# kepengxu/PGTFormer

Measured on NVIDIA H100. Metric: clips_per_s, higher is better.
Workload: dtype bf16

## Files before the change

pgtformer_b200/csrc/gemm_tc.cu:

```cuda
#include <cudaTypedefs.h>
#include <cstdio>
#include <cstdlib>

#include "common.cuh"
#include "tmap.cuh"
#include "ptx.cuh"
#include "epi_common.cuh"

namespace pgt {

constexpr int BM = 128;
constexpr int BK = 64;
constexpr int EPI_WARPS = 8;
constexpr int GEMM_THREADS = EPI_WARPS * 32 + 128;
constexpr int PRODUCER_WARP = EPI_WARPS;
constexpr int DMA_WARP = EPI_WARPS + 1;
constexpr int CONSUMER_REGS = 232;
constexpr int PRODUCER_REGS = 40;
static_assert(2 * 128 * CONSUMER_REGS + 128 * PRODUCER_REGS <= 65536, "register file");
constexpr int XCH_LD = 68;
constexpr int XCH_BYTES = BM * XCH_LD * 4;
constexpr int XCH_WG_LD = 36;
constexpr int XCH_WG_BYTES = BM * XCH_WG_LD * 4;
constexpr int EPI_BAR = 1;
constexpr int PP_XCH_BAR = 2;
constexpr int PP_MMA_BAR = 4;
constexpr int PP_EPI_BAR = 6;
constexpr int A_STAGE_BYTES = BM * BK * 2;
constexpr int PANEL_BYTES = BM * 128;
template <int BN>
constexpr int staging_slots() { return BN == 256 ? 2 : 4; }
constexpr int PREFETCH_TILES = 2;

enum { MODE_LINEAR = 0, MODE_CONV_S1 = 1, MODE_CONV_S2 = 2 };

struct GemmParams {
  int mode;
  int M, N, K;
  int num_kb, m_tiles, n_tiles;
  int F, H, W;
  int tw, th, tn, tiles_x, tiles_y;
  int cin_blocks, ksize, pad_lo, cin_ld;
  int pad_x, pad_y;
  long long o_sx, o_sy, o_sf;
  int b_resident;
  int fast_epi;
  int has_res_map;
  const float* bias;
  int act, epi_mode;
  float* gn_stats;
  int gn_cpg;
  int ntaps, tap_kw, tap_oy, tap_ox;
  int gn_tpf;
  int gn_fstride;
  int relu_after_res;
  const void* residual;
  int ldr, res_dtype;
  const void* aux;
  int ldaux;
  float sft_w;
  void* out;
  int ldo, out_dtype, out_layout;
  double flops;
};

template <int BN>
struct GemmCfg {
  static constexpr int B_STAGE_BYTES = BN * BK * 2;
  static constexpr int STAGE_BYTES = A_STAGE_BYTES + B_STAGE_BYTES;
  static constexpr int SLOTS = staging_slots<BN>();
  static constexpr int STAGING_BYTES = SLOTS * PANEL_BYTES;
  static constexpr int BUDGET = 232448 - 1024  - STAGING_BYTES - XCH_BYTES - 256 ;
  static constexpr int STAGES = (BUDGET / STAGE_BYTES) > 6 ? 6 : (BUDGET / STAGE_BYTES);
  static constexpr int SMEM_BYTES = STAGES * STAGE_BYTES + STAGING_BYTES + XCH_BYTES + 256 + 1024;
  static_assert(SMEM_BYTES <= 232448, "gemm smem budget");
};

__device__ __forceinline__ void tile_mn(const GemmParams& p, int tile, int& m_blk, int& n_blk) {
  n_blk = tile % p.n_tiles;
  m_blk = tile / p.n_tiles;
}


__device__ __forceinline__ void decode_conv_tile(const GemmParams& p, int m_blk, int& n0, int& y0, int& x0) {
  const int tx = m_blk % p.tiles_x;
  const int t2 = m_blk / p.tiles_x;
  const int ty = t2 % p.tiles_y;
  const int tf = t2 / p.tiles_y;
  x0 = tx * p.tw;
  y0 = ty * p.th;
  n0 = tf * p.tn;
}

template <int N>
__device__ __forceinline__ void act_chunk(float (&f)[N], int act) {
  switch (act) {
    case PGT_ACT_GELU:
#pragma unroll
      for (int j = 0; j < N; ++j) f[j] = gelu_erf(f[j]);
      break;
    case PGT_ACT_SILU:
#pragma unroll
      for (int j = 0; j < N; ++j) f[j] = apply_act(f[j], PGT_ACT_SILU);
      break;
    case PGT_ACT_LRELU02:
#pragma unroll
      for (int j = 0; j < N; ++j) f[j] = fmaxf(f[j], 0.2f * f[j]);
      break;
    case PGT_ACT_RELU:
#pragma unroll
      for (int j = 0; j < N; ++j) f[j] = fmaxf(f[j], 0.f);
      break;
    case PGT_ACT_SIGMOID:
#pragma unroll
      for (int j = 0; j < N; ++j) f[j] = apply_act(f[j], PGT_ACT_SIGMOID);
      break;
    default: break;
  }
}

struct EpiCtx {
  uint8_t* staging;
  float* xch;
  uint64_t* res_bar;
  uint64_t* slot_ready;
};

__device__ __forceinline__ uint4 lds128(uint32_t a) {
  uint4 u;
  asm volatile("ld.shared.v4.b32 {%0, %1, %2, %3}, [%4];" : "=r"(u.x), "=r"(u.y), "=r"(u.z), "=r"(u.w) : "r"(a) : "memory");
  return u;
}
__device__ __forceinline__ void sts128(uint32_t a, const uint4& u) {
  asm volatile("st.shared.v4.b32 [%0], {%1, %2, %3, %4};" ::"r"(a), "r"(u.x), "r"(u.y), "r"(u.z), "r"(u.w) : "memory");
}

template <bool kSft>
__device__ __forceinline__ void epi_finish(const GemmParams& p, const uint32_t (&v)[32], const float* bias32, uint32_t srow,
                                           int r, int sub, int esize, bool has_res, float* gq, int gcol,
                                           const float4 (&pre)[8], bool use_pre) {
  float f[32];
  if (use_pre) {
#pragma unroll
    for (int q = 0; q < 8; ++q) {
      f[4 * q + 0] = __uint_as_float(v[4 * q + 0]) + pre[q].x;
      f[4 * q + 1] = __uint_as_float(v[4 * q + 1]) + pre[q].y;
      f[4 * q + 2] = __uint_as_float(v[4 * q + 2]) + pre[q].z;
      f[4 * q + 3] = __uint_as_float(v[4 * q + 3]) + pre[q].w;
    }
  } else if (bias32 != nullptr) {
    const float4* b4 = reinterpret_cast<const float4*>(bias32);
#pragma unroll
    for (int q = 0; q < 8; ++q) {
      const float4 bb = __ldg(b4 + q);
      f[4 * q + 0] = __uint_as_float(v[4 * q + 0]) + bb.x;
      f[4 * q + 1] = __uint_as_float(v[4 * q + 1]) + bb.y;
      f[4 * q + 2] = __uint_as_float(v[4 * q + 2]) + bb.z;
      f[4 * q + 3] = __uint_as_float(v[4 * q + 3]) + bb.w;
    }
  } else {
#pragma unroll
    for (int i = 0; i < 32; ++i) f[i] = __uint_as_float(v[i]);
    if (p.bias != nullptr) {
#pragma unroll
      for (int i = 0; i < 32; ++i)
        if (gcol + i < p.N) f[i] += __ldg(p.bias + gcol + i);
    }
  }
  if (p.act != PGT_ACT_NONE && !p.relu_after_res) act_chunk(f, p.act);
  if (esize == 2) {
    uint32_t off[4];
#pragma unroll
    for (int q = 0; q < 4; ++q) off[q] = srow + ((((sub << 2) + q) ^ (r & 7)) << 4);
    if (has_res) {
      uint4 ur[4];
#pragma unroll
      for (int q = 0; q < 4; ++q) ur[q] = lds128(off[q]);
      if (kSft) {
        uint4 ux[4];
#pragma unroll
        for (int q = 0; q < 4; ++q) ux[q] = lds128(off[q] + PANEL_BYTES);
#pragma unroll
        for (int q = 0; q < 4; ++q) {
          const float2 a = unpack_bf16x2(ur[q].x), b = unpack_bf16x2(ur[q].y), c = unpack_bf16x2(ur[q].z), d = unpack_bf16x2(ur[q].w);
          const float rr[8] = {a.x, a.y, b.x, b.y, c.x, c.y, d.x, d.y};
          const float2 sa = unpack_bf16x2(ux[q].x), sb = unpack_bf16x2(ux[q].y), sc = unpack_bf16x2(ux[q].z), sd = unpack_bf16x2(ux[q].w);
          const float ss[8] = {sa.x, sa.y, sb.x, sb.y, sc.x, sc.y, sd.x, sd.y};
// ... 34 lines not shown
    }
  } else {
    if (has_res) {
      uint4 ur[8];
#pragma unroll
      for (int q = 0; q < 8; ++q) ur[q] = lds128(srow + ((q ^ (r & 7)) << 4));
#pragma unroll
      for (int q = 0; q < 8; ++q) {
        f[4 * q + 0] += __uint_as_float(ur[q].x); f[4 * q + 1] += __uint_as_float(ur[q].y);
        f[4 * q + 2] += __uint_as_float(ur[q].z); f[4 * q + 3] += __uint_as_float(ur[q].w);
      }
    }
    if (p.relu_after_res) {
#pragma unroll
      for (int e = 0; e < 32; ++e) f[e] = fmaxf(f[e], 0.f);
    }
#pragma unroll
    for (int q = 0; q < 8; ++q) {
      uint4 o;
      o.x = __float_as_uint(f[4 * q]); o.y = __float_as_uint(f[4 * q + 1]);
      o.z = __float_as_uint(f[4 * q + 2]); o.w = __float_as_uint(f[4 * q + 3]);
      sts128(srow + ((q ^ (r & 7)) << 4), o);
    }
  }
}

struct ItemCursor {
  int tile, pnl;
};

template <int BN>
struct ItemStream {
  const GemmParams& p;
  int num_tiles, PW, panels_total;
  __device__ ItemStream(const GemmParams& pp, int nt) : p(pp), num_tiles(nt) {
    PW = 128 / (pp.out_dtype == PGT_BF16 ? 2 : 4);
    panels_total = BN / PW;
  }
  __device__ int panels_in_tile(int t) const {
    int mb, nb;
    tile_mn(p, t, mb, nb);
    const int cb = nb * BN;
    const int n = (p.N - cb + PW - 1) / PW;
    return n > panels_total ? panels_total : n;
  }
  __device__ bool valid(const ItemCursor& c) const { return c.tile < num_tiles; }
  __device__ void next(ItemCursor& c) const {
    if (++c.pnl >= panels_in_tile(c.tile)) { c.tile += gridDim.x; c.pnl = 0; }
  }
};

template <int BN>
__device__ __forceinline__ void epilogue_dma_loop(const GemmParams& p, const EpiCtx& ctx, const CUtensorMap& tmO,
                                                  const CUtensorMap& tmR, const CUtensorMap& tmX, int lane, int num_tiles) {
  if (!p.fast_epi) return;
  const ItemStream<BN> is(p, num_tiles);
  constexpr int SLOTS = staging_slots<BN>();
  static_assert(SLOTS == 4 || SLOTS == 2, "ring positions are computed with shifts");
  const bool sft = SLOTS == 4 && p.epi_mode == PGT_EPI_SFT;
  const int S = sft ? 2 : 1;
  const int R = SLOTS / S;
  auto coords = [&](const ItemCursor& c, int& col, int& m_blk, int& n0, int& y0, int& x0) {
    int nb;
    tile_mn(p, c.tile, m_blk, nb);
    col = nb * BN + c.pnl * is.PW;
    n0 = y0 = x0 = 0;
    if (p.mode != MODE_LINEAR) decode_conv_tile(p, m_blk, n0, y0, x0);
  };
  auto prepare = [&](const ItemCursor& c, int pos) {
    uint64_t* bar = &ctx.res_bar[pos];
    if (!p.has_res_map) { mbar_arrive(bar); return; }
    int col, m_blk, n0, y0, x0;
    coords(c, col, m_blk, n0, y0, x0);
    uint8_t* dst = ctx.staging + pos * S * PANEL_BYTES;
    mbar_arrive_expect_tx(bar, S * PANEL_BYTES);
    if (p.mode == MODE_LINEAR) {
      tma_load_2d(dst, &tmR, bar, col, m_blk * BM);
      if (sft) tma_load_2d(dst + PANEL_BYTES, &tmX, bar, col, m_blk * BM);
    } else {
      tma_load_4d(dst, &tmR, bar, col, x0, y0, n0);
      if (sft) tma_load_4d(dst + PANEL_BYTES, &tmX, bar, col, x0, y0, n0);
    }
  };
  ItemCursor cp{(int)blockIdx.x, 0}, cs{(int)blockIdx.x, 0};
  if (lane == 0) {
    for (int i = 0; i < R && is.valid(cp); ++i) { prepare(cp, i); is.next(cp); }
  }
  __syncwarp();
  const int rshift = R == 4 ? 2 : 1;
  for (int k = 0; is.valid(cs); ++k, is.next(cs)) {
    const int pos = k & (R - 1);
    mbar_wait(&ctx.slot_ready[pos], (k >> rshift) & 1);
    if (lane == 0) {
      int col, m_blk, n0, y0, x0;
      coords(cs, col, m_blk, n0, y0, x0);
      const uint8_t* src = ctx.staging + pos * S * PANEL_BYTES;
      if (p.mode == MODE_LINEAR) tma_store_2d(&tmO, src, col, m_blk * BM);
      else tma_store_4d(&tmO, src, col, x0, y0, n0);
      bulk_commit();
      if (k >= 1 && is.valid(cp)) {
        bulk_wait_read<1>();
        prepare(cp, (k - 1) & (R - 1));
        is.next(cp);
      }
    }
    __syncwarp();
  }
  if (lane == 0) bulk_wait0();
}

struct DirectRow {
// ... 130 lines not shown
          mbar_wait_spin(&ctx.res_bar[pos], (k >> 1) & 1);
          const int col0 = col_base + pnl * PW + half * 32;
          uint32_t v[32];
          smem_row_32(xrow + half * 32, v);
          float4 nb[8];
          epi_finish<true>(p, v, bias_vec ? p.bias + col0 : nullptr, stg + pos * 2 * PANEL_BYTES, r, half, esize, true,
                           gn_ptr(col0), col0, nb, false);
          fence_proxy_async();
          mbar_arrive(&ctx.slot_ready[pos]);
          ++k;
        }
      } else {
        for (int pp = 0; pp < 64 / PW; ++pp) {
          const int pnl = g * (64 / PW) + pp;
          if (pnl >= npan) break;
          const int pos = k & (SLOTS - 1);
          const bool mine = (nsub == 2) || ((pnl & 1) == half);
          const int sb = (nsub == 2) ? half : 0;
          const int col0 = col_base + pnl * PW + sb * 32;
          float4 b[8];
          const bool pre = BN < 256 && bias_vec;
          if (mine && pre) {
            const float4* gb = reinterpret_cast<const float4*>(p.bias + col0);
#pragma unroll
            for (int q = 0; q < 8; ++q) b[q] = __ldg(gb + q);
          }
          mbar_wait_spin(&ctx.res_bar[pos], (k >> SLOT_SHIFT) & 1);
          if (mine) {
            uint32_t v[32];
            smem_row_32(xrow + pnl * PW + sb * 32 - g * 64, v);
            epi_finish<false>(p, v, bias_vec && !pre ? p.bias + col0 : nullptr, stg + pos * PANEL_BYTES, r, sb, esize,
                              p.has_res_map != 0, gn_ptr(col0), col0, b, pre);
          }
          fence_proxy_async();
          mbar_arrive(&ctx.slot_ready[pos]);
          ++k;
        }
      }
    } else {
      const int c0 = g * 64 + half * 32;
      if (drow.valid) {
#pragma unroll 1
        for (int sc16 = 0; sc16 < 32; sc16 += 16) {
          const int col0 = col_base + c0 + sc16;
          if (col0 >= p.N) break;
          epi_direct16<kVec>(p, drow, xrow + half * 32 + sc16, col0);
        }
      }
      __syncwarp();
    }
  });
}

template <int BN, bool kVec>
__device__ __forceinline__ void epilogue_tile_wg(const GemmParams& p, const EpiCtx& ctx, int wq, int bar, int tile, int k,
                                                 const float (&acc)[2][BN / 2]) {
  const int lane = lane_id();
  const int r = wq * 32 + lane;
  const int esize = (p.out_dtype == PGT_BF16) ? 2 : 4;
  const ItemStream<BN> is(p, 0);
  const int nsub = is.PW / 32;
  constexpr int SLOTS = staging_slots<BN>();
  constexpr int SLOT_SHIFT = SLOTS == 4 ? 2 : 1;
  const bool sft = SLOTS == 4 && p.epi_mode == PGT_EPI_SFT;
  const bool bias_vec = kVec && p.bias != nullptr && (p.N % 32) == 0;
  const float* xrow = ctx.xch + r * XCH_WG_LD;

  int n_blk, m_blk;
  tile_mn(p, tile, m_blk, n_blk);
  const int col_base = n_blk * BN;
  const int npan = p.fast_epi ? is.panels_in_tile(tile) : 0;
  const uint32_t stg = smem_u32(ctx.staging) + r * 128;
  const DirectRow drow = p.fast_epi ? DirectRow{false, 0, 0, 0, 0} : direct_row(p, m_blk, r);

  static_for<0, BN / 32>([&](auto cc) {
    constexpr int c = decltype(cc)::value;
    const int pnl = c / nsub, sub = c - pnl * nsub;
    if (p.fast_epi && pnl >= npan) return;
    const int col0 = col_base + c * 32;
    if (col0 < p.N) {
      named_bar_sync(bar, 128);
      acc_to_smem<c * 32, 32>(acc[0], ctx.xch, XCH_WG_LD, wq, lane);
      acc_to_smem<c * 32, 32>(acc[1], ctx.xch + 64 * XCH_WG_LD, XCH_WG_LD, wq, lane);
      named_bar_sync(bar, 128);
    }
    if (p.fast_epi) {
      const int item = k + pnl;
      const int pos = sft ? (item & 1) : (item & (SLOTS - 1));
      if (sub == 0) mbar_wait_spin(&ctx.res_bar[pos], sft ? ((item >> 1) & 1) : ((item >> SLOT_SHIFT) & 1));
      if (col0 < p.N) {
        uint32_t v[32];
        smem_row_32(xrow, v);
        float4 nb[8];
        if (sft)
          epi_finish<true>(p, v, bias_vec ? p.bias + col0 : nullptr, stg + pos * 2 * PANEL_BYTES, r, sub, esize, true,
                           gn_stats_ptr(p, m_blk, wq, col0), col0, nb, false);
        else
          epi_finish<false>(p, v, bias_vec ? p.bias + col0 : nullptr, stg + pos * PANEL_BYTES, r, sub, esize,
                            p.has_res_map != 0, gn_stats_ptr(p, m_blk, wq, col0), col0, nb, false);
      }
      if (sub == nsub - 1) {
        fence_proxy_async();
        mbar_arrive(&ctx.slot_ready[pos]);
      }
    } else if (col0 < p.N) {
      if (drow.valid) {
#pragma unroll 1
        for (int sc16 = 0; sc16 < 32; sc16 += 16) {
          if (col0 + sc16 >= p.N) break;
          epi_direct16<kVec>(p, drow, xrow + sc16, col0 + sc16);
        }
      }
      __syncwarp();
    }
  });
}

__device__ __forceinline__ void release_stage(uint64_t* bar, int lane) {
  __syncwarp();
  if (lane == 0) mbar_arrive(bar);
}

template <int BN, bool kVec>
__global__ void __launch_bounds__(GEMM_THREADS, 1)
gemm_tc_kernel(const __grid_constant__ CUtensorMap tmA, const __grid_constant__ CUtensorMap tmB,
               const __grid_constant__ CUtensorMap tmO, const __grid_constant__ CUtensorMap tmR,
               const __grid_constant__ CUtensorMap tmX, const GemmParams p) {
  using Cfg = GemmCfg<BN>;
  constexpr int STAGES = Cfg::STAGES;
  extern __shared__ uint8_t smem_raw[];
  uint8_t* smem = reinterpret_cast<uint8_t*>((reinterpret_cast<uintptr_t>(smem_raw) + 1023) & ~uintptr_t(1023));
  uint8_t* smem_a = smem;
  uint8_t* smem_b = smem + STAGES * A_STAGE_BYTES;
  uint8_t* staging = smem + STAGES * Cfg::STAGE_BYTES;
  float* xch = reinterpret_cast<float*>(staging + Cfg::STAGING_BYTES);
  uint64_t* bars = reinterpret_cast<uint64_t*>(staging + Cfg::STAGING_BYTES + XCH_BYTES);
  uint64_t* full_bar = bars;
  uint64_t* empty_bar = bars + STAGES;
  uint64_t* res_bar = bars + 2 * STAGES;
  uint64_t* slot_ready = res_bar + Cfg::SLOTS;

  const int warp = threadIdx.x >> 5;
  const int lane = threadIdx.x & 31;
  const int num_tiles = p.m_tiles * p.n_tiles;

  if (warp == PRODUCER_WARP && lane == 0) {
    tma_prefetch_desc(&tmA);
    tma_prefetch_desc(&tmB);
    if (p.fast_epi) tma_prefetch_desc(&tmO);
    if (p.has_res_map) tma_prefetch_desc(&tmR);
    if (p.fast_epi && p.epi_mode == PGT_EPI_SFT) tma_prefetch_desc(&tmX);
    for (int i = 0; i < STAGES; ++i) {
      mbar_init(&full_bar[i], 1);
      mbar_init(&empty_bar[i], EPI_WARPS);
    }
    for (int i = 0; i < Cfg::SLOTS; ++i) {
      mbar_init(&res_bar[i], 1);
      mbar_init(&slot_ready[i], EPI_WARPS * 32);
    }
    fence_barrier_init();
  }
  __syncthreads();

  if (warp >= EPI_WARPS) {
    setmaxnreg_dec<PRODUCER_REGS>();
    if (warp == PRODUCER_WARP) {
      int stage = 0;
      uint32_t phase = 0;
      for (int tile = blockIdx.x; tile < num_tiles; tile += gridDim.x) {
        int n_blk, m_blk;
        tile_mn(p, tile, m_blk, n_blk);
        int n0 = 0, y0 = 0, x0 = 0;
        if (p.mode != MODE_LINEAR) decode_conv_tile(p, m_blk, n0, y0, x0);
        for (int kb = 0; kb < p.num_kb; ++kb) {
          mbar_wait(&empty_bar[stage], phase ^ 1);
          if (elect_one()) {
            void* dst_a = smem_a + stage * A_STAGE_BYTES;
            void* dst_b = smem_b + stage * Cfg::B_STAGE_BYTES;
            int cb = 0, ax = 0, ay = 0, a5 = 0;
            if (p.mode != MODE_LINEAR) {
              const int tap = kb / p.cin_blocks;
              cb = kb - tap * p.cin_blocks;
              const int dy = tap / p.ksize;
              const int dx = tap - dy * p.ksize;
              if (p.mode == MODE_CONV_S1) {
                ax = x0 + dx - p.pad_x; ay = y0 + dy - p.pad_y;
              } else {
                const int oy = dy - p.pad_lo, ox = dx - p.pad_lo;
                const int qy = (oy < 0) ? -((1 - oy) >> 1) : (oy >> 1);
                const int qx = (ox < 0) ? -((1 - ox) >> 1) : (ox >> 1);
                const int py = oy - 2 * qy, px = ox - 2 * qx;
                cb = px * p.cin_ld + cb * BK;
                ax = x0 + qx; ay = y0 + qy; a5 = py;
              }
            }
            mbar_arrive_expect_tx(&full_bar[stage], Cfg::STAGE_BYTES);
            if (p.mode == MODE_LINEAR) tma_load_2d(dst_a, &tmA, &full_bar[stage], kb * BK, m_blk * BM);
            else if (p.mode == MODE_CONV_S1) tma_load_4d(dst_a, &tmA, &full_bar[stage], cb * BK, ax, ay, n0);
            else tma_load_5d(dst_a, &tmA, &full_bar[stage], cb, ax, a5, ay, n0);
            tma_load_2d(dst_b, &tmB, &full_bar[stage], kb * BK, n_blk * BN);
          }
          __syncwarp();
          if (++stage == STAGES) { stage = 0; phase ^= 1; }
        }
      }
      for (int i = 0; i < STAGES; ++i) {
        mbar_wait(&empty_bar[stage], phase ^ 1);
        if (++stage == STAGES) { stage = 0; phase ^= 1; }
      }
    } else if (warp == DMA_WARP) {
      const EpiCtx ctx{staging, xch, res_bar, slot_ready};
      epilogue_dma_loop<BN>(p, ctx, tmO, tmR, tmX, lane, num_tiles);
    }
  } else {
    setmaxnreg_inc<CONSUMER_REGS>();
    const EpiCtx ctx{staging, xch, res_bar, slot_ready};
    const int wg = warp >> 2;
    const uint32_t a_rows = smem_u32(smem_a) + wg * 64 * 128;
    const uint32_t b_base = smem_u32(smem_b);
    int stage = 0;
    uint32_t phase = 0;
    int k = 0;
    for (int tile = blockIdx.x; tile < num_tiles; tile += gridDim.x) {
      float acc[BN / 2];
      int prev = -1;
      for (int kb = 0; kb < p.num_kb; ++kb) {
        mbar_wait_spin(&full_bar[stage], phase);
        const uint64_t da = wgmma_desc_k_sw128(a_rows + stage * A_STAGE_BYTES);
        const uint64_t db = wgmma_desc_k_sw128(b_base + stage * Cfg::B_STAGE_BYTES);
        wgmma_fence();
#pragma unroll
        for (int kk = 0; kk < BK / 16; ++kk)
          wgmma_bf16<BN>(acc, da + 2 * kk, db + 2 * kk, (kb | kk) != 0 ? 1u : 0u);
        wgmma_commit();
        wgmma_wait<1>();
        if (prev >= 0) release_stage(&empty_bar[prev], lane);
        prev = stage;
        if (++stage == STAGES) { stage = 0; phase ^= 1; }
      }
      wgmma_wait<0>();
      release_stage(&empty_bar[prev], lane);
      epilogue_tile<BN, kVec>(p, ctx, warp, lane, tile, k, acc);
    }
  }
}


constexpr int HALO_TW = 8, HALO_TH = 16;
constexpr int HALO_PITCH = (HALO_TW + 2) * 128;
constexpr int HALO_A_BYTES = (HALO_TH + 2) * HALO_PITCH;
constexpr int HALO_A_STRIDE = ((HALO_A_BYTES + 1023) / 1024) * 1024;

template <int BN>
struct HaloCfg {
  static constexpr int B_BYTES = BN * 128;
  static constexpr int A_STAGES = 2;
  static constexpr int B_STAGES = (BN == 64) ? 9 : 4;
  static constexpr int SLOTS = staging_slots<BN>();
  static constexpr int STAGING_BYTES = SLOTS * PANEL_BYTES;
  static constexpr int XCH = 2 * XCH_WG_BYTES;
  static constexpr int SMEM_BYTES = A_STAGES * HALO_A_STRIDE + B_STAGES * B_BYTES + STAGING_BYTES + XCH + 512 + 1024;
  static_assert(SMEM_BYTES <= 232448, "halo conv smem budget");
};

template <int S>
__device__ __forceinline__ void ring_skip(int& s, uint32_t& ph, int n) {
  const int t = s + n;
  ph ^= (uint32_t)(t / S) & 1u;
  s = t % S;
}

template <int BN, bool kVec>
__global__ void __launch_bounds__(GEMM_THREADS, 1)
conv_halo_kernel(const __grid_constant__ CUtensorMap tmA, const __grid_constant__ CUtensorMap tmB,
                 const __grid_constant__ CUtensorMap tmO, const __grid_constant__ CUtensorMap tmR,
                 const __grid_constant__ CUtensorMap tmX, const GemmParams p) {
  using Cfg = HaloCfg<BN>;
  constexpr int AS = Cfg::A_STAGES, BS = Cfg::B_STAGES;
  constexpr int RELEASERS = 4;
  extern __shared__ uint8_t smem_raw[];
  uint8_t* smem = reinterpret_cast<uint8_t*>((reinterpret_cast<uintptr_t>(smem_raw) + 1023) & ~uintptr_t(1023));
  uint8_t* smem_a = smem;
  uint8_t* smem_b = smem + AS * HALO_A_STRIDE;
  uint8_t* staging = smem_b + BS * Cfg::B_BYTES;
  float* xch = reinterpret_cast<float*>(staging + Cfg::STAGING_BYTES);
  uint64_t* bars = reinterpret_cast<uint64_t*>(staging + Cfg::STAGING_BYTES + Cfg::XCH);
  uint64_t* a_full = bars;
  uint64_t* a_empty = bars + AS;
  uint64_t* b_full = bars + 2 * AS;
  uint64_t* b_empty = bars + 2 * AS + BS;
  uint64_t* res_bar = bars + 2 * AS + 2 * BS;
  uint64_t* slot_ready = res_bar + Cfg::SLOTS;

  const int warp = threadIdx.x >> 5;
  const int lane = threadIdx.x & 31;
  const int num_tiles = p.m_tiles * p.n_tiles;
  const int cin_pad = p.cin_blocks * BK;

  if (warp == PRODUCER_WARP && lane == 0) {
    tma_prefetch_desc(&tmA);
    tma_prefetch_desc(&tmB);
    if (p.fast_epi) tma_prefetch_desc(&tmO);
    if (p.has_res_map) tma_prefetch_desc(&tmR);
    if (p.fast_epi && p.epi_mode == PGT_EPI_SFT) tma_prefetch_desc(&tmX);
    for (int i = 0; i < AS; ++i) { mbar_init(&a_full[i], 1); mbar_init(&a_empty[i], RELEASERS); }
    for (int i = 0; i < BS; ++i) { mbar_init(&b_full[i], 1); mbar_init(&b_empty[i], RELEASERS); }
    for (int i = 0; i < Cfg::SLOTS; ++i) {
      mbar_init(&res_bar[i], 1);
      mbar_init(&slot_ready[i], RELEASERS * 32);
    }
    fence_barrier_init();
  }
  __syncthreads();

  if (warp >= EPI_WARPS) {
    setmaxnreg_dec<PRODUCER_REGS>();
    if (warp == PRODUCER_WARP) {
      int as = 0, bs = 0;
      uint32_t aph = 0, bph = 0;
      for (int tile = blockIdx.x; tile < num_tiles; tile += gridDim.x) {
        const int n_blk = tile % p.n_tiles;
        const int m_blk = tile / p.n_tiles;
        int n0, y0, x0;
        decode_conv_tile(p, m_blk, n0, y0, x0);
        {
          const int pt = tile + PREFETCH_TILES * (int)gridDim.x;
          if (BN == 64 && pt < num_tiles && elect_one()) {
            int pn0, py0, px0;
            decode_conv_tile(p, pt / p.n_tiles, pn0, py0, px0);
            for (int cb = 0; cb < p.cin_blocks; ++cb) tma_prefetch_4d(&tmA, cb * BK, px0 - 1, py0 - 1, pn0);
            if (p.has_res_map) {
              const int c0 = (pt % p.n_tiles) * BN;
              const int rw = p.out_dtype == PGT_BF16 ? 64 : 32;
              for (int c = 0; c < BN && c0 + c < p.N; c += rw) {
                tma_prefetch_4d(&tmR, c0 + c, px0, py0, pn0);
                if (p.epi_mode == PGT_EPI_SFT) tma_prefetch_4d(&tmX, c0 + c, px0, py0, pn0);
              }
            }
          }
          __syncwarp();
        }
        for (int cb = 0; cb < p.cin_blocks; ++cb) {
          mbar_wait(&a_empty[as], aph ^ 1);
          if (elect_one()) {
            mbar_arrive_expect_tx(&a_full[as], HALO_A_BYTES);
            tma_load_4d(smem_a + as * HALO_A_STRIDE, &tmA, &a_full[as], cb * BK, x0 - 1, y0 - 1, n0);
          }
          __syncwarp();
          if (++as == AS) { as = 0; aph ^= 1; }
          if (p.b_resident && tile != (int)blockIdx.x) continue;
          for (int t = 0; t < p.ntaps; ++t) {
            mbar_wait(&b_empty[bs], bph ^ 1);
            if (elect_one()) {
              mbar_arrive_expect_tx(&b_full[bs], Cfg::B_BYTES);
              tma_load_2d(smem_b + bs * Cfg::B_BYTES, &tmB, &b_full[bs], t * cin_pad + cb * BK, n_blk * BN);
            }
            __syncwarp();
            if (++bs == BS) { bs = 0; bph ^= 1; }
          }
        }
      }
      for (int i = 0; i < AS; ++i) {
        mbar_wait(&a_empty[as], aph ^ 1);
        if (++as == AS) { as = 0; aph ^= 1; }
      }
    } else if (warp == DMA_WARP) {
      const EpiCtx ctx{staging, xch, res_bar, slot_ready};
      epilogue_dma_loop<BN>(p, ctx, tmO, tmR, tmX, lane, num_tiles);
    }
  } else {
    setmaxnreg_inc<CONSUMER_REGS>();
    const int wg = warp >> 2;
    const EpiCtx ctx{staging, xch + wg * (XCH_WG_BYTES / 4), res_bar, slot_ready};
    const uint32_t a_base = smem_u32(smem_a);
    const uint32_t b_base = smem_u32(smem_b);
    constexpr uint64_t ROW_BLOCK = 8 * HALO_PITCH / 16;
    const ItemStream<BN> is(p, num_tiles);
    const int b_per_tile = p.b_resident ? 0 : p.ntaps * p.cin_blocks;
    int as = 0, bs = 0;
    uint32_t aph = 0, bph = 0;
    int k = 0;
    bool first = true;
    for (int tile = blockIdx.x, j = 0; tile < num_tiles; tile += gridDim.x, ++j) {
      const bool has_next = tile + (int)gridDim.x < num_tiles;
      const int items = p.fast_epi ? is.panels_in_tile(tile) : 0;
      if ((j & 1) != wg) {
        ring_skip<AS>(as, aph, p.cin_blocks);
        ring_skip<BS>(bs, bph, b_per_tile);
        k += items;
        continue;
      }
      if (j > 0) named_bar_sync(PP_MMA_BAR + wg, 256);
      float acc[2][BN / 2];
      for (int cb = 0; cb < p.cin_blocks; ++cb) {
        const bool hand_over = has_next && cb == p.cin_blocks - 1;
        mbar_wait_spin(&a_full[as], aph);
        const uint64_t da0 = wgmma_desc_k_sw128(a_base + as * HALO_A_STRIDE, HALO_PITCH);
        auto tap_desc = [&](int t) -> uint64_t {
          const int dy = t / p.tap_kw, dx = t - dy * p.tap_kw;
          return da0 + (uint64_t)(((dy + p.tap_oy) * (HALO_TW + 2) + dx + p.tap_ox) * 8);
        };
        if (p.b_resident && first) {
          for (int t = 0; t < p.ntaps * p.cin_blocks; ++t) mbar_wait_spin(&b_full[t], 0);
          first = false;
        }
        int prev = -1;
        for (int t = 0; t < p.ntaps; ++t) {
          int bst = cb * p.ntaps + t;
          if (!p.b_resident) {
            mbar_wait_spin(&b_full[bs], bph);
            bst = bs;
          }
          const uint64_t da = tap_desc(t);
          const uint64_t db = wgmma_desc_k_sw128(b_base + bst * Cfg::B_BYTES);
          wgmma_fence();
#pragma unroll
          for (int kk = 0; kk < BK / 16; ++kk) {
            const uint32_t accum = (cb | t | kk) != 0 ? 1u : 0u;
            wgmma_bf16<BN>(acc[0], da + 2 * kk, db + 2 * kk, accum);
            wgmma_bf16<BN>(acc[1], da + ROW_BLOCK + 2 * kk, db + 2 * kk, accum);
          }
          wgmma_commit();
          if (hand_over && t == p.ntaps - 1) named_bar_arrive(PP_MMA_BAR + (wg ^ 1), 256);
          wgmma_wait<1>();
          if (!p.b_resident) {
            if (prev >= 0) release_stage(&b_empty[prev], lane);
            prev = bs;
            if (++bs == BS) { bs = 0; bph ^= 1; }
          }
        }
        wgmma_wait<0>();
        if (!p.b_resident) release_stage(&b_empty[prev], lane);
        release_stage(&a_empty[as], lane);
        if (++as == AS) { as = 0; aph ^= 1; }
      }
      if (j > 0) named_bar_sync(PP_EPI_BAR + wg, 256);
      epilogue_tile_wg<BN, kVec>(p, ctx, warp & 3, PP_XCH_BAR + wg, tile, k, acc);
      if (has_next) named_bar_arrive(PP_EPI_BAR + (wg ^ 1), 256);
      k += items;
    }
  }
}

static int encode_map(CUtensorMap* map, const void* base, int rank, const uint64_t* dims, const uint64_t* strides_bytes,
                      const uint32_t* box, int dtype = PGT_BF16) {
  return tmap_encode(map, base, rank, dims, strides_bytes, box, dtype);
}

static inline bool aligned16(const void* p) { return (reinterpret_cast<uintptr_t>(p) & 15) == 0; }

static int encode_out_map(CUtensorMap* map, const GemmParams& p, const void* base, int ld, int dtype) {
  const int esize = dtype == PGT_BF16 ? 2 : 4;
  const uint32_t pw = 128 / esize;
  if (p.mode == MODE_LINEAR) {
    uint64_t dims[2] = {(uint64_t)p.N, (uint64_t)p.M};
    uint64_t str[1] = {(uint64_t)ld * esize};
    uint32_t box[2] = {pw, BM};
    return encode_map(map, base, 2, dims, str, box, dtype);
  }
  uint64_t dims[4] = {(uint64_t)p.N, (uint64_t)p.W, (uint64_t)p.H, (uint64_t)p.F};
  uint64_t str[3] = {(uint64_t)ld * esize, (uint64_t)p.W * ld * esize, (uint64_t)p.H * p.W * ld * esize};
  if (p.o_sx != 0 && base == p.out) {
    str[0] = (uint64_t)p.o_sx * esize; str[1] = (uint64_t)p.o_sy * esize; str[2] = (uint64_t)p.o_sf * esize;
  }
  uint32_t box[4] = {pw, (uint32_t)p.tw, (uint32_t)p.th, (uint32_t)p.tn};
  return encode_map(map, base, 4, dims, str, box, dtype);
}

static int setup_epilogue_maps(GemmParams& p, const CUtensorMap& placeholder, CUtensorMap& tmO, CUtensorMap& tmR,
                               CUtensorMap& tmX) {
  const int esize = p.out_dtype == PGT_BF16 ? 2 : 4;
  p.fast_epi = (p.out_layout == PGT_OUT_NHWC && aligned16(p.out) && ((long long)p.ldo * esize) % 16 == 0) ? 1 : 0;
  if (p.epi_mode == PGT_EPI_SFT &&
      !(p.out_dtype == PGT_BF16 && aligned16(p.aux) && ((long long)p.ldaux * 2) % 16 == 0 && p.o_sx == 0))
    p.fast_epi = 0;
  p.has_res_map = 0;
  if (p.fast_epi && p.residual != nullptr) {
    if (p.res_dtype == p.out_dtype && aligned16(p.residual) && ((long long)p.ldr * esize) % 16 == 0) p.has_res_map = 1;
    else p.fast_epi = 0;
  }
  if (p.gn_stats != nullptr) {
    const int cpg = p.N / 32;
    const bool ok = p.fast_epi && p.out_dtype == PGT_BF16 && (p.N % 32) == 0 &&
                    (cpg == 2 || cpg == 4 || cpg == 8 || cpg == 16 || cpg == 32) &&
                    (p.mode == MODE_LINEAR || p.tn == 1);
    if (!ok) return PGT_ERR_UNSUPPORTED;
    p.gn_cpg = cpg;
  }
  tmO = placeholder;
  tmR = placeholder;
  tmX = placeholder;
  if (p.fast_epi) {
    int rc = encode_out_map(&tmO, p, p.out, p.ldo, p.out_dtype);
    if (rc != PGT_OK) return rc;
    if (p.has_res_map) {
      rc = encode_out_map(&tmR, p, p.residual, p.ldr, p.res_dtype);
      if (rc != PGT_OK) return rc;
    }
    if (p.epi_mode == PGT_EPI_SFT) {
      if (!p.has_res_map) { p.fast_epi = 0; return p.gn_stats ? PGT_ERR_UNSUPPORTED : PGT_OK; }
      rc = encode_out_map(&tmX, p, p.aux, p.ldaux, PGT_BF16);
      if (rc != PGT_OK) return rc;
    }
  }
  return PGT_OK;
}

static bool vector_views(const GemmParams& p) {
  if (p.bias != nullptr && (p.N % 32) == 0 && !aligned16(p.bias)) return false;
  if (!p.fast_epi && p.out_layout == PGT_OUT_NHWC && p.out_dtype == PGT_BF16 && (p.ldo % 8) == 0 && !aligned16(p.out))
    return false;
  return true;
}

template <int BN, bool kVec>
static cudaError_t gemm_smem_once() {
  static PerDeviceOnce once;
  return once.run([] {
    return cudaFuncSetAttribute(gemm_tc_kernel<BN, kVec>, cudaFuncAttributeMaxDynamicSharedMemorySize, GemmCfg<BN>::SMEM_BYTES);
  });
}

template <int BN, bool kVec>
static cudaError_t halo_smem_once() {
  static PerDeviceOnce once;
  return once.run([] {
    return cudaFuncSetAttribute(conv_halo_kernel<BN, kVec>, cudaFuncAttributeMaxDynamicSharedMemorySize, HaloCfg<BN>::SMEM_BYTES);
  });
}

static int encode_weight_map(CUtensorMap* tmB, const void* W, int ldw, int K, int N, int BN) {
  uint64_t dims[2] = {(uint64_t)K, (uint64_t)N};
  uint64_t str[1] = {(uint64_t)ldw * 2};
  uint32_t box[2] = {BK, (uint32_t)BN};
  return encode_map(tmB, W, 2, dims, str, box);
}

template <int BN>
static int launch_gemm(const CUtensorMap& tmA, const void* W, int ldw, GemmParams& p, cudaStream_t stream) {
  using Cfg = GemmCfg<BN>;
  static_assert(Cfg::STAGES >= 3, "pipeline too shallow");
  CUtensorMap tmB, tmO, tmR, tmX;
  int rc = encode_weight_map(&tmB, W, ldw, p.K, p.N, BN);
  if (rc != PGT_OK) return rc;
  rc = setup_epilogue_maps(p, tmA, tmO, tmR, tmX);
  if (rc != PGT_OK) return rc;
  p.n_tiles = ceil_div(p.N, BN);
  const bool vec = vector_views(p);
  PGT_CUDA_OK((vec ? gemm_smem_once<BN, true>() : gemm_smem_once<BN, false>()));
  const int tiles = p.m_tiles * p.n_tiles;
  const int grid = tiles < num_sms() ? tiles : num_sms();
  {
    char desc[96];
    if (prof_enabled()) {
      if (p.mode == MODE_LINEAR) snprintf(desc, sizeof(desc), "linear M%d N%d K%d BN%d e%d", p.M, p.N, p.K, BN, p.fast_epi);
      else snprintf(desc, sizeof(desc), "conv%d s%d F%d H%d W%d K%d N%d BN%d t%dx%dx%d e%d", p.ksize, p.mode, p.F, p.H, p.W, p.K, p.N, BN, p.tn, p.th, p.tw, p.fast_epi);
    }
    ProfScope ps(PGT_PROF_GEMM, p.flops, stream, desc);
    if (vec) gemm_tc_kernel<BN, true><<<grid, GEMM_THREADS, Cfg::SMEM_BYTES, stream>>>(tmA, tmB, tmO, tmR, tmX, p);
    else gemm_tc_kernel<BN, false><<<grid, GEMM_THREADS, Cfg::SMEM_BYTES, stream>>>(tmA, tmB, tmO, tmR, tmX, p);
  }
  PGT_LAUNCH_OK();
  return PGT_OK;
}

template <int BN>
static int launch_halo(const CUtensorMap& tmA, const void* W, int ldw, GemmParams& p, cudaStream_t stream) {
  using Cfg = HaloCfg<BN>;
  CUtensorMap tmB, tmO, tmR, tmX;
  int rc = encode_weight_map(&tmB, W, ldw, p.K, p.N, BN);
  if (rc != PGT_OK) return rc;
  rc = setup_epilogue_maps(p, tmA, tmO, tmR, tmX);
  if (rc != PGT_OK) return rc;
  p.n_tiles = ceil_div(p.N, BN);
  p.b_resident = (p.ntaps * p.cin_blocks <= Cfg::B_STAGES && p.n_tiles == 1) ? 1 : 0;
  const bool vec = vector_views(p);
  PGT_CUDA_OK((vec ? halo_smem_once<BN, true>() : halo_smem_once<BN, false>()));
  const int tiles = p.m_tiles * p.n_tiles;
  const int grid = tiles < num_sms() ? tiles : num_sms();
  {
    char desc[96];
    if (prof_enabled())
      snprintf(desc, sizeof(desc), "halo3 F%d H%d W%d K%d N%d BN%d e%d r%d", p.F, p.H, p.W, p.K, p.N, BN, p.fast_epi,
               p.b_resident);
    ProfScope ps(PGT_PROF_GEMM, p.flops, stream, desc);
    if (vec) conv_halo_kernel<BN, true><<<grid, GEMM_THREADS, Cfg::SMEM_BYTES, stream>>>(tmA, tmB, tmO, tmR, tmX, p);
    else conv_halo_kernel<BN, false><<<grid, GEMM_THREADS, Cfg::SMEM_BYTES, stream>>>(tmA, tmB, tmO, tmR, tmX, p);
  }
  PGT_LAUNCH_OK();
  return PGT_OK;
}

static bool wide_tiles(const GemmParams& p) {
  if (p.N <= 128 || p.num_kb < 8 || p.epi_mode == PGT_EPI_SFT) return false;
  if (ceil_div(p.N, 256) * 256 > ceil_div(p.N, 128) * 128) return false;
  return p.m_tiles * ceil_div(p.N, 256) >= num_sms();
}

static int dispatch_gemm(const CUtensorMap& tmA, const void* W, int ldw, GemmParams& p, cudaStream_t stream) {
  if (p.N <= 64) return launch_gemm<64>(tmA, W, ldw, p, stream);
  if (wide_tiles(p)) return launch_gemm<256>(tmA, W, ldw, p, stream);
  return launch_gemm<128>(tmA, W, ldw, p, stream);
}

static int fill_epilogue(GemmParams& p, const pgt_epilogue* ep) {
  if (ep == nullptr || ep->out == nullptr) return PGT_ERR_INVALID;
  p.bias = ep->bias;
  p.act = ep->act;
  p.epi_mode = ep->mode;
  p.residual = ep->residual;
  p.ldr = ep->ldr;
  p.res_dtype = ep->res_dtype;
  p.aux = ep->aux;
// ... 173 lines not shown
```

Before: 90.47.

## Add register-fragment epilogue using stmatrix/ldmatrix into staging, dropping fp32 exchange buffer

Adds a fast-epilogue path in which the consumer warps apply bias, activation and residual/SFT straight from wgmma accumulator fragments. They read residuals with ldmatrix or 64-bit shared loads and write results into the swizzled TMA staging panels with stmatrix, skipping the fp32 exchange buffer. Freeing the exchange buffer lets this variant use four staging slots and possibly more pipeline stages, and the shared-memory layout is reordered to put barriers first. The old exchange path is kept for the slow epilogue and for GroupNorm statistics. The risks are extra template instantiations and subtle swizzle/indexing correctness in the new fragment mapping.

```diff
diff --git a/pgtformer_b200/csrc/gemm_tc.cu b/pgtformer_b200/csrc/gemm_tc.cu
--- a/pgtformer_b200/csrc/gemm_tc.cu
+++ b/pgtformer_b200/csrc/gemm_tc.cu
@@ -68,12 +68,17 @@
 struct GemmCfg {
   static constexpr int B_STAGE_BYTES = BN * BK * 2;
   static constexpr int STAGE_BYTES = A_STAGE_BYTES + B_STAGE_BYTES;
-  static constexpr int SLOTS = staging_slots<BN>();
-  static constexpr int STAGING_BYTES = SLOTS * PANEL_BYTES;
-  static constexpr int BUDGET = 232448 - 1024  - STAGING_BYTES - XCH_BYTES - 256 ;
-  static constexpr int STAGES = (BUDGET / STAGE_BYTES) > 6 ? 6 : (BUDGET / STAGE_BYTES);
-  static constexpr int SMEM_BYTES = STAGES * STAGE_BYTES + STAGING_BYTES + XCH_BYTES + 256 + 1024;
-  static_assert(SMEM_BYTES <= 232448, "gemm smem budget");
+  static constexpr int AVAIL = 232448 - 1024  - 1024 ;
+  static constexpr int stages_for(int rest) { return (rest / STAGE_BYTES) > 6 ? 6 : (rest / STAGE_BYTES); }
+  static constexpr int SLOTS_XCH = staging_slots<BN>();
+  static constexpr int STAGES_XCH = stages_for(AVAIL - SLOTS_XCH * PANEL_BYTES - XCH_BYTES);
+  static constexpr int SMEM_XCH = STAGES_XCH * STAGE_BYTES + SLOTS_XCH * PANEL_BYTES + XCH_BYTES + 1024 + 1024;
+  static constexpr int SLOTS_FRAG = 4;
+  static constexpr int STAGES_FRAG = stages_for(AVAIL - SLOTS_FRAG * PANEL_BYTES);
+  static constexpr int SMEM_FRAG = STAGES_FRAG * STAGE_BYTES + SLOTS_FRAG * PANEL_BYTES + 1024 + 1024;
+  static_assert(SMEM_XCH <= 232448 && SMEM_FRAG <= 232448, "gemm smem budget");
+  static_assert(STAGES_XCH >= 3 && STAGES_FRAG >= 3, "pipeline too shallow");
+  static_assert(STAGES_XCH <= 6 && STAGES_FRAG <= 6, "barrier area");
 };
 
 __device__ __forceinline__ void tile_mn(const GemmParams& p, int tile, int& m_blk, int& n_blk) {
@@ -273,11 +278,10 @@
 
 template <int BN>
 __device__ __forceinline__ void epilogue_dma_loop(const GemmParams& p, const EpiCtx& ctx, const CUtensorMap& tmO,
-                                                  const CUtensorMap& tmR, const CUtensorMap& tmX, int lane, int num_tiles) {
+                                                  const CUtensorMap& tmR, const CUtensorMap& tmX, int lane, int num_tiles,
+                                                  int SLOTS) {
   if (!p.fast_epi) return;
   const ItemStream<BN> is(p, num_tiles);
-  constexpr int SLOTS = staging_slots<BN>();
-  static_assert(SLOTS == 4 || SLOTS == 2, "ring positions are computed with shifts");
   const bool sft = SLOTS == 4 && p.epi_mode == PGT_EPI_SFT;
   const int S = sft ? 2 : 1;
   const int R = SLOTS / S;
@@ -578,29 +582,177 @@
   });
 }
 
+__device__ __forceinline__ void ldsm_x4(uint32_t a, uint32_t* u) {
+  asm volatile("ldmatrix.sync.aligned.m8n8.x4.shared.b16 {%0, %1, %2, %3}, [%4];"
+               : "=r"(u[0]), "=r"(u[1]), "=r"(u[2]), "=r"(u[3]) : "r"(a) : "memory");
+}
+__device__ __forceinline__ void stsm_x4(uint32_t a, uint32_t u0, uint32_t u1, uint32_t u2, uint32_t u3) {
+  asm volatile("stmatrix.sync.aligned.m8n8.x4.shared.b16 [%0], {%1, %2, %3, %4};" ::"r"(a), "r"(u0), "r"(u1), "r"(u2),
+               "r"(u3) : "memory");
+}
+__device__ __forceinline__ uint2 lds64(uint32_t a) {
+  uint2 u;
+  asm volatile("ld.shared.v2.b32 {%0, %1}, [%2];" : "=r"(u.x), "=r"(u.y) : "r"(a) : "memory");
+  return u;
+}
+__device__ __forceinline__ void sts64(uint32_t a, uint2 u) {
+  asm volatile("st.shared.v2.b32 [%0], {%1, %2};" ::"r"(a), "r"(u.x), "r"(u.y) : "memory");
+}
+
+template <int BN, bool kVec>
+__device__ __forceinline__ void epilogue_tile_frag(const GemmParams& p, const EpiCtx& ctx, int tile, int& k,
+                                                   const float (&acc)[BN / 2]) {
+  constexpr int SLOTS = GemmCfg<BN>::SLOTS_FRAG;
+  const int warp = threadIdx.x >> 5;
+  const int lane = lane_id();
+  const int r0 = (warp >> 2) * 64 + (warp & 3) * 16 + (lane >> 2);
+  const int t = lane & 3;
+  const int sw = lane >> 2;
+  const int mrow = r0 - (lane >> 2) + 8 * ((lane >> 3) & 1) + (lane & 7);
+  const ItemStream<BN> is(p, 0);
+  const bool sft = p.epi_mode == PGT_EPI_SFT;
+  const bool has_res = p.has_res_map != 0;
+  const bool bias_vec = kVec && p.bias != nullptr && (p.N % 32) == 0;
+  int n_blk, m_blk;
+  tile_mn(p, tile, m_blk, n_blk);
+  const int col_base = n_blk * BN;
+  const int npan = is.panels_in_tile(tile);
+  const uint32_t row0 = smem_u32(ctx.staging) + r0 * 128;
+  auto bias2 = [&](int c) -> float2 {
+    if (bias_vec) return __ldg(reinterpret_cast<const float2*>(p.bias + c));
+    return make_float2(c < p.N ? __ldg(p.bias + c) : 0.f, c + 1 < p.N ? __ldg(p.bias + c + 1) : 0.f);
+  };
+  auto wait_slot = [&](int& pos) {
+    pos = sft ? (k & 1) : (k & (SLOTS - 1));
+    mbar_wait_spin(&ctx.res_bar[pos], sft ? ((k >> 1) & 1) : ((k >> 2) & 1));
+  };
+  auto signal_slot = [&](int pos) {
+    fence_proxy_async();
+    mbar_arrive(&ctx.slot_ready[pos]);
+    ++k;
+  };
+
+  if (p.out_dtype == PGT_BF16) {
+    static_for<0, BN / 64>([&](auto gc) {
+      constexpr int g = decltype(gc)::value;
+      if (g >= npan) return;
+      int pos = 0;
+      static_for<0, 2>([&](auto hc) {
+        constexpr int hh = decltype(hc)::value;
+        float f[16];
+#pragma unroll
+        for (int i = 0; i < 16; ++i) f[i] = acc[32 * g + 16 * hh + i];
+        if (p.bias != nullptr) {
+#pragma unroll
+          for (int jj = 0; jj < 4; ++jj) {
+            const float2 b = bias2(col_base + 64 * g + 8 * (4 * hh + jj) + 2 * t);
+            f[4 * jj + 0] += b.x; f[4 * jj + 1] += b.y; f[4 * jj + 2] += b.x; f[4 * jj + 3] += b.y;
+          }
+        }
+        if (p.act != PGT_ACT_NONE && !p.relu_after_res) act_chunk(f, p.act);
+        if (hh == 0) wait_slot(pos);
+        const uint32_t m0 = smem_u32(ctx.staging) + pos * (sft ? 2 : 1) * PANEL_BYTES + mrow * 128;
+        auto moff = [&](int pr) { return m0 + (((4 * hh + 2 * pr + (lane >> 4)) ^ (lane & 7)) << 4); };
+        if (has_res) {
+          uint32_t ur[8];
+          ldsm_x4(moff(0), ur);
+          ldsm_x4(moff(1), ur + 4);
+          if (sft) {
+            uint32_t ux[8];
+            ldsm_x4(moff(0) + PANEL_BYTES, ux);
+            ldsm_x4(moff(1) + PANEL_BYTES, ux + 4);
+#pragma unroll
+            for (int h = 0; h < 8; ++h) {
+              const float2 rr = unpack_bf16x2(ur[h]), ss = unpack_bf16x2(ux[h]);
+              f[2 * h + 0] = rr.x + p.sft_w * (rr.x * ss.x + f[2 * h + 0]);
+              f[2 * h + 1] = rr.y + p.sft_w * (rr.y * ss.y + f[2 * h + 1]);
+            }
+          } else {
+#pragma unroll
+            for (int h = 0; h < 8; ++h) {
+              const float2 rr = unpack_bf16x2(ur[h]);
+              f[2 * h + 0] += rr.x; f[2 * h + 1] += rr.y;
+            }
+          }
+        }
+        if (p.relu_after_res) {
+#pragma unroll
+          for (int e = 0; e < 16; ++e) f[e] = fmaxf(f[e], 0.f);
+        }
+#pragma unroll
+        for (int pr = 0; pr < 2; ++pr)
+          stsm_x4(moff(pr), pack_bf16x2(f[8 * pr + 0], f[8 * pr + 1]), pack_bf16x2(f[8 * pr + 2], f[8 * pr + 3]),
+                  pack_bf16x2(f[8 * pr + 4], f[8 * pr + 5]), pack_bf16x2(f[8 * pr + 6], f[8 * pr + 7]));
+      });
+      signal_slot(pos);
+    });
+  } else {
+    static_for<0, BN / 32>([&](auto qc) {
+      constexpr int q = decltype(qc)::value;
+      if (q >= npan) return;
+      float f[16];
+#pragma unroll
+      for (int i = 0; i < 16; ++i) f[i] = acc[16 * q + i];
+      if (p.bias != nullptr) {
+#pragma unroll
+        for (int j = 0; j < 4; ++j) {
+          const float2 b = bias2(col_base + 32 * q + 8 * j + 2 * t);
+          f[4 * j + 0] += b.x; f[4 * j + 1] += b.y; f[4 * j + 2] += b.x; f[4 * j + 3] += b.y;
+        }
+      }
+      if (p.act != PGT_ACT_NONE && !p.relu_after_res) act_chunk(f, p.act);
+      int pos;
+      wait_slot(pos);
+      const uint32_t a0 = row0 + pos * PANEL_BYTES + (t & 1) * 8;
+      uint32_t off[4];
+#pragma unroll
+      for (int j = 0; j < 4; ++j) off[j] = a0 + (((2 * j + (t >> 1)) ^ sw) << 4);
+      if (has_res) {
+        uint2 ur[8];
+#pragma unroll
+        for (int j = 0; j < 4; ++j) { ur[2 * j] = lds64(off[j]); ur[2 * j + 1] = lds64(off[j] + 8 * 128); }
+#pragma unroll
+        for (int h = 0; h < 8; ++h) { f[2 * h + 0] += __uint_as_float(ur[h].x); f[2 * h + 1] += __uint_as_float(ur[h].y); }
+      }
+      if (p.relu_after_res) {
+#pragma unroll
+        for (int e = 0; e < 16; ++e) f[e] = fmaxf(f[e], 0.f);
+      }
+#pragma unroll
+      for (int j = 0; j < 4; ++j) {
+        sts64(off[j], make_uint2(__float_as_uint(f[4 * j + 0]), __float_as_uint(f[4 * j + 1])));
+        sts64(off[j] + 8 * 128, make_uint2(__float_as_uint(f[4 * j + 2]), __float_as_uint(f[4 * j + 3])));
+      }
+      signal_slot(pos);
+    });
+  }
+}
+
 __device__ __forceinline__ void release_stage(uint64_t* bar, int lane) {
   __syncwarp();
   if (lane == 0) mbar_arrive(bar);
 }
 
-template <int BN, bool kVec>
+template <int BN, bool kVec, bool kXch>
 __global__ void __launch_bounds__(GEMM_THREADS, 1)
 gemm_tc_kernel(const __grid_constant__ CUtensorMap tmA, const __grid_constant__ CUtensorMap tmB,
                const __grid_constant__ CUtensorMap tmO, const __grid_constant__ CUtensorMap tmR,
                const __grid_constant__ CUtensorMap tmX, const GemmParams p) {
   using Cfg = GemmCfg<BN>;
-  constexpr int STAGES = Cfg::STAGES;
+  constexpr bool use_xch = kXch;
+  constexpr int STAGES = use_xch ? Cfg::STAGES_XCH : Cfg::STAGES_FRAG;
+  constexpr int slots = use_xch ? Cfg::SLOTS_XCH : Cfg::SLOTS_FRAG;
   extern __shared__ uint8_t smem_raw[];
   uint8_t* smem = reinterpret_cast<uint8_t*>((reinterpret_cast<uintptr_t>(smem_raw) + 1023) & ~uintptr_t(1023));
-  uint8_t* smem_a = smem;
-  uint8_t* smem_b = smem + STAGES * A_STAGE_BYTES;
-  uint8_t* staging = smem + STAGES * Cfg::STAGE_BYTES;
-  float* xch = reinterpret_cast<float*>(staging + Cfg::STAGING_BYTES);
-  uint64_t* bars = reinterpret_cast<uint64_t*>(staging + Cfg::STAGING_BYTES + XCH_BYTES);
+  uint64_t* bars = reinterpret_cast<uint64_t*>(smem);
   uint64_t* full_bar = bars;
-  uint64_t* empty_bar = bars + STAGES;
-  uint64_t* res_bar = bars + 2 * STAGES;
-  uint64_t* slot_ready = res_bar + Cfg::SLOTS;
+  uint64_t* empty_bar = bars + 6;
+  uint64_t* res_bar = bars + 12;
+  uint64_t* slot_ready = bars + 16;
+  uint8_t* staging = smem + 1024;
+  uint8_t* smem_a = staging + slots * PANEL_BYTES;
+  uint8_t* smem_b = smem_a + STAGES * A_STAGE_BYTES;
+  float* xch = reinterpret_cast<float*>(smem_b + STAGES * Cfg::B_STAGE_BYTES);
 
   const int warp = threadIdx.x >> 5;
   const int lane = threadIdx.x & 31;
@@ -616,7 +768,7 @@
       mbar_init(&full_bar[i], 1);
       mbar_init(&empty_bar[i], EPI_WARPS);
     }
-    for (int i = 0; i < Cfg::SLOTS; ++i) {
+    for (int i = 0; i < slots; ++i) {
       mbar_init(&res_bar[i], 1);
       mbar_init(&slot_ready[i], EPI_WARPS * 32);
     }
@@ -672,7 +824,7 @@
       }
     } else if (warp == DMA_WARP) {
       const EpiCtx ctx{staging, xch, res_bar, slot_ready};
-      epilogue_dma_loop<BN>(p, ctx, tmO, tmR, tmX, lane, num_tiles);
+      epilogue_dma_loop<BN>(p, ctx, tmO, tmR, tmX, lane, num_tiles, slots);
     }
   } else {
     setmaxnreg_inc<CONSUMER_REGS>();
@@ -696,13 +848,14 @@
           wgmma_bf16<BN>(acc, da + 2 * kk, db + 2 * kk, (kb | kk) != 0 ? 1u : 0u);
         wgmma_commit();
         wgmma_wait<1>();
-        if (prev >= 0) release_stage(&empty_bar[prev], lane);
+        if (prev >= 0) release_stage(&empty_bar[prev], lane_id());
         prev = stage;
         if (++stage == STAGES) { stage = 0; phase ^= 1; }
       }
       wgmma_wait<0>();
-      release_stage(&empty_bar[prev], lane);
-      epilogue_tile<BN, kVec>(p, ctx, warp, lane, tile, k, acc);
+      release_stage(&empty_bar[prev], lane_id());
+      if constexpr (use_xch) epilogue_tile<BN, kVec>(p, ctx, threadIdx.x >> 5, lane_id(), tile, k, acc);
+      else epilogue_tile_frag<BN, kVec>(p, ctx, tile, k, acc);
     }
   }
 }
@@ -828,7 +981,7 @@
       }
     } else if (warp == DMA_WARP) {
       const EpiCtx ctx{staging, xch, res_bar, slot_ready};
-      epilogue_dma_loop<BN>(p, ctx, tmO, tmR, tmX, lane, num_tiles);
+      epilogue_dma_loop<BN>(p, ctx, tmO, tmR, tmX, lane, num_tiles, Cfg::SLOTS);
     }
   } else {
     setmaxnreg_inc<CONSUMER_REGS>();
@@ -975,11 +1128,12 @@
   return true;
 }
 
-template <int BN, bool kVec>
+template <int BN, bool kVec, bool kXch>
 static cudaError_t gemm_smem_once() {
   static PerDeviceOnce once;
   return once.run([] {
-    return cudaFuncSetAttribute(gemm_tc_kernel<BN, kVec>, cudaFuncAttributeMaxDynamicSharedMemorySize, GemmCfg<BN>::SMEM_BYTES);
+    return cudaFuncSetAttribute(gemm_tc_kernel<BN, kVec, kXch>, cudaFuncAttributeMaxDynamicSharedMemorySize,
+                                kXch ? GemmCfg<BN>::SMEM_XCH : GemmCfg<BN>::SMEM_FRAG);
   });
 }
 
@@ -1001,15 +1155,17 @@
 template <int BN>
 static int launch_gemm(const CUtensorMap& tmA, const void* W, int ldw, GemmParams& p, cudaStream_t stream) {
   using Cfg = GemmCfg<BN>;
-  static_assert(Cfg::STAGES >= 3, "pipeline too shallow");
   CUtensorMap tmB, tmO, tmR, tmX;
   int rc = encode_weight_map(&tmB, W, ldw, p.K, p.N, BN);
   if (rc != PGT_OK) return rc;
   rc = setup_epilogue_maps(p, tmA, tmO, tmR, tmX);
   if (rc != PGT_OK) return rc;
   p.n_tiles = ceil_div(p.N, BN);
+  const bool xch = !p.fast_epi || p.gn_stats != nullptr;
+  const int smem = xch ? Cfg::SMEM_XCH : Cfg::SMEM_FRAG;
   const bool vec = vector_views(p);
-  PGT_CUDA_OK((vec ? gemm_smem_once<BN, true>() : gemm_smem_once<BN, false>()));
+  PGT_CUDA_OK((vec ? (xch ? gemm_smem_once<BN, true, true>() : gemm_smem_once<BN, true, false>())
+                   : (xch ? gemm_smem_once<BN, false, true>() : gemm_smem_once<BN, false, false>())));
   const int tiles = p.m_tiles * p.n_tiles;
   const int grid = tiles < num_sms() ? tiles : num_sms();
   {
@@ -1019,8 +1175,9 @@
       else snprintf(desc, sizeof(desc), "conv%d s%d F%d H%d W%d K%d N%d BN%d t%dx%dx%d e%d", p.ksize, p.mode, p.F, p.H, p.W, p.K, p.N, BN, p.tn, p.th, p.tw, p.fast_epi);
     }
     ProfScope ps(PGT_PROF_GEMM, p.flops, stream, desc);
-    if (vec) gemm_tc_kernel<BN, true><<<grid, GEMM_THREADS, Cfg::SMEM_BYTES, stream>>>(tmA, tmB, tmO, tmR, tmX, p);
-    else gemm_tc_kernel<BN, false><<<grid, GEMM_THREADS, Cfg::SMEM_BYTES, stream>>>(tmA, tmB, tmO, tmR, tmX, p);
+    auto kernel = vec ? (xch ? gemm_tc_kernel<BN, true, true> : gemm_tc_kernel<BN, true, false>)
+                      : (xch ? gemm_tc_kernel<BN, false, true> : gemm_tc_kernel<BN, false, false>);
+    kernel<<<grid, GEMM_THREADS, smem, stream>>>(tmA, tmB, tmO, tmR, tmX, p);
   }
   PGT_LAUNCH_OK();
   return PGT_OK;
```

Result: faster. 92.03 (median of 6 runs) (+1.7%).

## Swap operands for BN=64 halo conv to issue one m64n128 wgmma

Applied to the files above, without the earlier changes.

For the BN=64 halo conv kernel, the weight tile becomes the wgmma A operand and the 128-pixel activation tile the B operand, so each k-step issues a single m64n128k16 instruction instead of two m64n64 instructions. A new transposed accumulator-to-shared path writes the swapped fragment into the exchange buffer for the existing epilogue. This halves the wgmma instruction count and may use the tensor cores better at small N. The risk is that the halo activation layout must be valid as a K-major B descriptor with the tap offsets, and the transposed stores may cost more in the epilogue.

```diff
diff --git a/pgtformer_b200/csrc/gemm_tc.cu b/pgtformer_b200/csrc/gemm_tc.cu
--- a/pgtformer_b200/csrc/gemm_tc.cu
+++ b/pgtformer_b200/csrc/gemm_tc.cu
@@ -133,6 +133,9 @@
 }
 __device__ __forceinline__ void sts128(uint32_t a, const uint4& u) {
   asm volatile("st.shared.v4.b32 [%0], {%1, %2, %3, %4};" ::"r"(a), "r"(u.x), "r"(u.y), "r"(u.z), "r"(u.w) : "memory");
+}
+__device__ __forceinline__ void sts32(uint32_t a, float v) {
+  asm volatile("st.shared.f32 [%0], %1;" ::"r"(a), "f"(v) : "memory");
 }
 
 template <bool kSft>
@@ -514,9 +517,31 @@
   });
 }
 
-template <int BN, bool kVec>
+template <int C0, int N>
+__device__ __forceinline__ void acc_to_xch(const float (&acc)[2][N], float* xch, int wq, int lane) {
+  acc_to_smem<C0, 32>(acc[0], xch, XCH_WG_LD, wq, lane);
+  acc_to_smem<C0, 32>(acc[1], xch + 64 * XCH_WG_LD, XCH_WG_LD, wq, lane);
+}
+template <int C0>
+__device__ __forceinline__ void acc_to_xch(const float (&d)[64], float* xch, int wq, int lane) {
+  static_assert(C0 == 0 || C0 == 32, "a 32-row chunk of the m64 fragment");
+  static_assert(XCH_WG_LD % 32 == 4, "conflict-free transposed stores");
+  if ((wq >> 1) != C0 / 32) return;
+  constexpr uint32_t LD = XCH_WG_LD * 4;
+  const uint32_t x0 = smem_u32(xch) + (2 * (lane & 3) * XCH_WG_LD + 16 * (wq & 1) + (lane >> 2)) * 4;
+#pragma unroll
+  for (int j = 0; j < 16; ++j) {
+    const uint32_t x = x0 + 8 * j * LD;
+    sts32(x, d[4 * j + 0]);
+    sts32(x + LD, d[4 * j + 1]);
+    sts32(x + 32, d[4 * j + 2]);
+    sts32(x + LD + 32, d[4 * j + 3]);
+  }
+}
+
+template <int BN, bool kVec, typename Acc>
 __device__ __forceinline__ void epilogue_tile_wg(const GemmParams& p, const EpiCtx& ctx, int wq, int bar, int tile, int k,
-                                                 const float (&acc)[2][BN / 2]) {
+                                                 const Acc& acc) {
   const int lane = lane_id();
   const int r = wq * 32 + lane;
   const int esize = (p.out_dtype == PGT_BF16) ? 2 : 4;
@@ -542,8 +567,7 @@
     const int col0 = col_base + c * 32;
     if (col0 < p.N) {
       named_bar_sync(bar, 128);
-      acc_to_smem<c * 32, 32>(acc[0], ctx.xch, XCH_WG_LD, wq, lane);
-      acc_to_smem<c * 32, 32>(acc[1], ctx.xch + 64 * XCH_WG_LD, XCH_WG_LD, wq, lane);
+      acc_to_xch<c * 32>(acc, ctx.xch, wq, lane);
       named_bar_sync(bar, 128);
     }
     if (p.fast_epi) {
@@ -723,6 +747,7 @@
   static constexpr int XCH = 2 * XCH_WG_BYTES;
   static constexpr int SMEM_BYTES = A_STAGES * HALO_A_STRIDE + B_STAGES * B_BYTES + STAGING_BYTES + XCH + 512 + 1024;
   static_assert(SMEM_BYTES <= 232448, "halo conv smem budget");
+  using Acc = std::conditional_t<BN == 64, float[64], float[2][BN / 2]>;
 };
 
 template <int S>
@@ -853,7 +878,7 @@
         continue;
       }
       if (j > 0) named_bar_sync(PP_MMA_BAR + wg, 256);
-      float acc[2][BN / 2];
+      typename Cfg::Acc acc;
       for (int cb = 0; cb < p.cin_blocks; ++cb) {
         const bool hand_over = has_next && cb == p.cin_blocks - 1;
         mbar_wait_spin(&a_full[as], aph);
@@ -873,14 +898,18 @@
             mbar_wait_spin(&b_full[bs], bph);
             bst = bs;
           }
-          const uint64_t da = tap_desc(t);
-          const uint64_t db = wgmma_desc_k_sw128(b_base + bst * Cfg::B_BYTES);
+          const uint64_t dx = tap_desc(t);
+          const uint64_t dw = wgmma_desc_k_sw128(b_base + bst * Cfg::B_BYTES);
           wgmma_fence();
 #pragma unroll
           for (int kk = 0; kk < BK / 16; ++kk) {
             const uint32_t accum = (cb | t | kk) != 0 ? 1u : 0u;
-            wgmma_bf16<BN>(acc[0], da + 2 * kk, db + 2 * kk, accum);
-            wgmma_bf16<BN>(acc[1], da + ROW_BLOCK + 2 * kk, db + 2 * kk, accum);
+            if constexpr (BN == 64) {
+              wgmma_bf16<128>(acc, dw + 2 * kk, dx + 2 * kk, accum);
+            } else {
+              wgmma_bf16<BN>(acc[0], dx + 2 * kk, dw + 2 * kk, accum);
+              wgmma_bf16<BN>(acc[1], dx + ROW_BLOCK + 2 * kk, dw + 2 * kk, accum);
+            }
           }
           wgmma_commit();
           if (hand_over && t == p.ntaps - 1) named_bar_arrive(PP_MMA_BAR + (wg ^ 1), 256);
```

After: 90.08 before, 90.67 after, median of 6. No clear change (+0.7%).
